# febrianrachmadi/dep-gan-im

Measured on AMD Instinct MI355X. Metric: 2D slices/sec (G+2D+GP train step), 256x256x1 fp32, higher is better.
Workload: dtype f32; 1 GPU; DEP-GAN-IM twoCritics canonical train step (critic-Y2 + critic-DEM + G update, WGAN-GP), batch 32 per GPU, 256x256x1; per_gpu_batch=32, global_batch=32, parallelism=dp1

## Files before the change

dep_gan_im_amd/_lib.py:

```python
from __future__ import annotations

import ctypes as C
import os

HERE = os.path.dirname(os.path.abspath(__file__))
LIB_PATH = os.environ.get("DEPGAN_LIB") or os.path.join(HERE, "libdepgan.so")

EXPORTS = [
    "depgan_last_error", "depgan_create", "depgan_destroy", "depgan_set_stream", "depgan_param_count",
    "depgan_param_info", "depgan_arena_floats", "depgan_arena_ptr", "depgan_weights_changed", "depgan_g_forward",
    "depgan_d_forward", "depgan_critic_grads", "depgan_critic_step", "depgan_g_eval", "depgan_g_grads",
    "depgan_g_step", "depgan_apply_adam", "depgan_last_sums", "depgan_profile_enable", "depgan_profile_read",
    "depgan_profile_reset", "depgan_profile_dump", "depgan_op_conv2d", "depgan_op_conv2d_bwd_data", "depgan_op_conv2d_wgrad",
    "depgan_op_maxpool", "depgan_op_deconv2x2", "depgan_op_deconv2x2_wgrad", "depgan_op_conv2d_stamps", "depgan_uresnet_grads", "depgan_uresnet_step",
    "depgan_uresnet_eval", "depgan_profile_read_bytes", "depgan_g_eval_multi", "depgan_eval_accumulate", "depgan_eval_counts",
    "depgan_data_prep_scratch_floats", "depgan_data_prep_subject", "depgan_abi_version", "depgan_config_size",
    "depgan_set_allreduce", "depgan_get_adam_step", "depgan_set_adam_step", "depgan_gen_iteration", "depgan_eval_divide",
    "depgan_source_hash", "depgan_debug_capture", "depgan_debug_tensor", "depgan_rccl_unique_id", "depgan_rccl_init",
    "depgan_rccl_broadcast", "depgan_rccl_info", "depgan_rccl_shutdown", "depgan_op_conv2d_wgrad_bf16",
    "depgan_op_bn_moments", "depgan_op_bn_backward", "depgan_op_affine_act", "depgan_op_softmax_ce4",
    "depgan_op_bn_rows_fwd", "depgan_op_bn_rows_bwd", "depgan_op_small_gemm",
    "depgan_op_unpool_mask", "depgan_op_gather_pool", "depgan_op_head", "depgan_op_critic_tail_fwd",
    "depgan_op_critic_tail_bwd", "depgan_op_critic_tail_wgrad", "depgan_op_colsum", "depgan_op_sum",
    "depgan_op_critic_inputs", "depgan_op_gp_u0", "depgan_op_critic_stats", "depgan_op_gloss_sums", "depgan_op_g_dpre",
    "depgan_op_film_bwd", "depgan_op_bn_prepare_batch", "depgan_op_bn_gamma_grad_batch", "depgan_op_noise_fwd",
    "depgan_op_noise_bwd", "depgan_op_best_noise", "depgan_op_round_bf16_masked",
    "depgan_data_zscore_scratch_floats", "depgan_data_prep_zscore", "depgan_data_mask_slices", "depgan_labels_to_onehot",
    "depgan_eval_accumulate_channels", "depgan_eval_label_counts",
    "depgan_g_forward_bf16s", "depgan_debug_tensor_bf16s", "depgan_op_conv2d_bf16s", "depgan_op_deconv2x2_bf16s",
    "depgan_op_edge_conv_bf16s", "depgan_op_head_bf16s",
    "depgan_set_fwd_only_storage", "depgan_get_fwd_only_storage", "depgan_op_conv2d_head_bf16s",
    "depgan_set_g_update_storage", "depgan_get_g_update_storage", "depgan_debug_film_decision_bf16s",
    "depgan_op_conv2d_film_train_bf16s", "depgan_op_conv2d_wgrad_bf16s", "depgan_op_conv2d_bwd_data_bf16s",
    "depgan_op_unpool_mask_bf16s", "depgan_op_film_bwd_bf16s", "depgan_op_head_bwd_bf16s",
    "depgan_op_conv2d_fused", "depgan_op_deconv2x2_igemm", "depgan_op_conv2d_wgrad_ex",
    "depgan_set_critic16_pipe", "depgan_get_critic16_pipe", "depgan_op_head_softmax_bf16s",
]

ABI_VERSION = 3
MAX_MULTI, MAX_CRITIC_STEPS = 32, 256
RCCL_ID_BYTES = 128


class Config(C.Structure):
    _fields_ = [("struct_size", C.c_int), ("batch", C.c_int), ("height", C.c_int), ("width", C.c_int),
                ("nicg", C.c_int), ("first_fm", C.c_int), ("im_thresh", C.c_float), ("delta", C.c_float),
                ("lrD", C.c_float), ("lrG", C.c_float), ("beta1", C.c_float), ("beta2", C.c_float),
                ("adam_eps", C.c_float), ("nc_out", C.c_int), ("bf16_weights", C.c_int), ("bf16_mfma", C.c_int),
                ("f32_split", C.c_int)]

    def __init__(self, **kw):
        super().__init__(**kw)
        self.struct_size = C.sizeof(Config)


ALLREDUCE_FN = C.CFUNCTYPE(C.c_int, C.c_void_p, C.c_void_p, C.c_long, C.c_void_p)


NET_G, NET_D_Y2, NET_D_DEM = 0, 1, 2
ARENA_PARAMS, ARENA_NONTRAINABLE, ARENA_GRADS, ARENA_ADAM_M, ARENA_ADAM_V = range(5)

_lib = None


class DepganError(RuntimeError):
    pass


def load():
# ... 99 lines not shown
    lib.depgan_op_g_dpre.argtypes = [vp, i] + [vp] * 5 + [i, L, vp]
    lib.depgan_op_film_bwd.argtypes = [vp] * 4 + [i] + [vp] * 3 + [i, L, i, L, vp]
    lib.depgan_op_bn_prepare_batch.argtypes = [vp, vp, i, f, vp]
    lib.depgan_op_bn_gamma_grad_batch.argtypes = [vp, vp, i, vp]
    lib.depgan_op_noise_fwd.argtypes = [vp] * 6 + [i, vp]
    lib.depgan_op_noise_bwd.argtypes = [vp] * 10 + [i, L, vp]
    lib.depgan_op_best_noise.argtypes = [vp, i, vp, L, vp, vp, vp]
    lib.depgan_op_round_bf16_masked.argtypes = [vp] * 3 + [L, vp]
    lib.depgan_uresnet_grads.argtypes = [vp, vp, vp, vp, C.c_int, C.c_uint, fp]
    lib.depgan_uresnet_step.argtypes = [vp, vp, vp, vp, C.c_int, C.c_uint, fp]
    lib.depgan_uresnet_eval.argtypes = [vp, vp, vp, vp, C.c_int, fp]
    lib.depgan_debug_capture.argtypes = [vp, C.c_int]
    lib.depgan_rccl_unique_id.argtypes = [vp]
    lib.depgan_rccl_init.argtypes = [vp, vp, C.c_int, C.c_int]
    lib.depgan_rccl_broadcast.argtypes = [vp, vp, C.c_long, C.c_int]
    lib.depgan_rccl_info.argtypes = [vp, ip, ip, C.POINTER(C.c_long)]
    lib.depgan_rccl_shutdown.argtypes = [vp]
    lib.depgan_debug_tensor.argtypes = [vp, C.c_char_p, vp, C.c_long, ip]
    lib.depgan_g_forward_bf16s.argtypes = [vp, vp, vp, vp, i]
    lib.depgan_debug_tensor_bf16s.argtypes = [vp, C.c_char_p, vp, L, ip]
    lib.depgan_op_conv2d_bf16s.argtypes = [vp, L, L, L] + [vp] * 6 + [i] + [vp, L, L, L] * 2 + [vp] + [i] * 7 + [vp]
    lib.depgan_op_deconv2x2_bf16s.argtypes = [vp, L, L, L] + [vp] * 4 + [vp, L, L, L] + [i] * 6 + [vp]
    lib.depgan_op_edge_conv_bf16s.argtypes = [vp] * 5 + [vp, L, L, L] + [i] * 6 + [vp]
    lib.depgan_op_head_bf16s.argtypes = [vp] * 4 + [L, i, i, vp]
    lib.depgan_op_head_softmax_bf16s.argtypes = [vp, L] + [vp] * 4 + [L, i, vp]
    lib.depgan_op_conv2d_head_bf16s.argtypes = ([vp, L, L, L] + [vp] * 6 + [i] + [vp, L, L, L] * 2 + [vp] + [i] * 7 +
                                                [vp] * 3 + [i, i, vp])
    lib.depgan_set_fwd_only_storage.argtypes = [vp, i]
    lib.depgan_get_fwd_only_storage.argtypes = [vp]
    lib.depgan_set_g_update_storage.argtypes = [vp, i]
    lib.depgan_get_g_update_storage.argtypes = [vp]
    lib.depgan_set_critic16_pipe.argtypes = [vp, i]
    lib.depgan_get_critic16_pipe.argtypes = [vp]
    lib.depgan_debug_film_decision_bf16s.argtypes = [vp, C.c_char_p, vp, L, ip]
    lib.depgan_op_conv2d_film_train_bf16s.argtypes = ([vp, L, L, L] + [vp] * 6 + [i] + [vp, L, L, L] * 2 + [vp, vp] +
                                                      [i] * 6 + [vp])
    lib.depgan_op_conv2d_wgrad_bf16s.argtypes = [vp, L, L, L] * 2 + [vp, vp] + [i] * 7 + [vp]
    lib.depgan_op_conv2d_bwd_data_bf16s.argtypes = [vp, L, L, L] + [vp] + [vp, L, L, L] * 3 + [i] * 6 + [vp]
    lib.depgan_op_unpool_mask_bf16s.argtypes = [vp, L, L, L] * 4 + [i] * 4 + [vp]
    lib.depgan_op_film_bwd_bf16s.argtypes = [vp] * 4 + [i] + [vp] * 3 + [i, L, i, vp]
    lib.depgan_op_head_bwd_bf16s.argtypes = [i, vp, L] + [vp] * 3 + [L, i, vp]
    lib.depgan_op_conv2d_fused.argtypes = ([vp, L, L, L] + [vp] * 6 + [i] + [vp, L, L, L] * 5 + [vp] * 3 + [i] * 12 +
                                           [vp])
    lib.depgan_op_deconv2x2_igemm.argtypes = [i] + [vp, L, L, L] + [vp] * 4 + [vp, L, L, L] * 2 + [i] * 7 + [vp]
    lib.depgan_op_conv2d_wgrad_ex.argtypes = [vp, L, L, L] * 2 + [vp] * 3 + [i] * 3 + [vp] * 3 + [i] * 7 + [vp]
    _lib = lib
    return lib


def check(rc, what=""):
    if rc != 0:
        msg = load().depgan_last_error()
        raise DepganError("%s failed (status %d): %s" % (what or "libdepgan call", rc,
                                                         msg.decode() if msg else "?"))


_hip = None


def hip():
    global _hip
    if _hip is None:
        last = None
        for name in ("libamdhip64.so", "/opt/rocm/lib/libamdhip64.so", "libamdhip64.so.7", "libamdhip64.so.6"):
            try:
                _hip = C.CDLL(name)
# ... 18 lines not shown
```

dep_gan_im_amd/csrc/common.h:

```cpp
#pragma once
#include <hip/hip_runtime.h>
#include <stdint.h>
#include <stddef.h>

typedef float f32x2 __attribute__((ext_vector_type(2)));
typedef float f32x4 __attribute__((ext_vector_type(4)));
typedef float f32x16 __attribute__((ext_vector_type(16)));

struct TView {
  float* p;
  long sB, sY, sX;
};

static inline TView make_view(float* p, int H, int W, int C) {
  TView v;
  v.p = p;
  v.sX = C;
  v.sY = (long)W * C;
  v.sB = (long)H * W * C;
  return v;
}
static inline TView make_view_slice(float* p, int H, int W, int Ctot, int c0) {
  TView v = make_view(p, H, W, Ctot);
  v.p = p + c0;
// ... 181 lines not shown
  float* dst;
  const float* kscale;
  int ntaps, srcI, srcO, io, transpose, flip;
  int NT, CK, nCC, Kdim, Ndim;
  int bf16;
  int tapg;
  int wino;
  unsigned total;
  unsigned per_nt;
  unsigned nt_stride;
  unsigned blk0, nblk;
};
int dg_pack_job(const ConvPlan& pl, const float* src, int srcI, int srcO, int io, int transpose, int flip,
                const float* kscale, float* dst, size_t nt_stride, PackJob* job);
unsigned dg_pack_layout(PackJob* jobs_host, int njobs);
int dg_pack_weights_batch(const PackJob* jobs_dev, int njobs, unsigned nblocks, hipStream_t st);

int dg_pack_weights(const ConvPlan& pl, const float* src, int srcI, int srcO, int io, int transpose, int flip,
                    const float* kscale, float* dst, hipStream_t st);

int dg_conv_igemm(const ConvPlan& pl, const ConvArgs& a, hipStream_t st);
int dg_conv_igemm_check(const ConvPlan& pl, const ConvArgs& a);
bool dg_conv_igemm_wp_supported(const ConvPlan& pl, const ConvArgs& a, bool force);
int dg_conv_igemm_wp(const ConvPlan& pl, const ConvArgs& a, hipStream_t st);
bool dg_conv_igemm_ws5_supported(const ConvPlan& pl, const ConvArgs& a, bool force);
int dg_conv_igemm_ws5(const ConvPlan& pl, const ConvArgs& a, hipStream_t st);
const char* dg_conv_igemm_ws5_name(const ConvPlan& pl);
int dg_conv_igemm_tile(const ConvPlan& pl, const ConvArgs& a, hipStream_t st);
bool dg_conv_igemm_head_supported(const ConvPlan& pl, const ConvArgs& a);
ConvPlan dg_plan_conv_wino(int Cin, int Cout);
bool dg_conv_wino_supported(const ConvPlan& pl, const ConvArgs& a);
const char* dg_conv_wino_name(const ConvArgs& a);
int dg_conv_wino(const ConvPlan& pl, const ConvArgs& a, hipStream_t st);
void dg_conv_igemm_name(const ConvPlan& pl, const ConvArgs& a, char* buf, size_t cap);
int dg_conv_direct(int KS, const ConvArgs& a, hipStream_t st);

size_t dg_wgrad_part_floats(int KS, int B, int H, int W, int Cin, int Cout);
int dg_wgrad(int KS, const WgradArgs& a, int* nchunks, hipStream_t st);
int dg_wgrad_finish(const float* part, int nchunks, int ntaps, int Cin, int Cout, const float* scale, float* out,
                    float* raw, int accumulate, int oi, const float* colpart, int colC, const float* colscale,
                    float* colout, float* colraw, hipStream_t st);
int dg_wgrad_finish_rows(const float* part, int nchunks, int ntaps, int Cin, int Cout, const float* scale, float* out,
                         float* raw, int accumulate, int oi, const float* colpart, int colrows, int colC,
                         const float* colscale, float* colout, float* colraw, hipStream_t st);
int dg_wgrad_reduce(const float* part, int nchunks, int ntaps, int Cin, int Cout, const float* scale, float* out,
                    float* raw, int accumulate, int oi, hipStream_t st);

bool dg_wgrad_bf16_supported(int KS, int Cin, int Cout);
size_t dg_wgrad_bf16_part_floats(int KS, int B, int H, int W, int Cin, int Cout);
int dg_wgrad_bf16(int KS, const WgradArgs& a, int* nchunks, hipStream_t st);

size_t dg_wgrad_small_part_floats(int KS, int B, int H, int W, int Cin, int Cout);
int dg_wgrad_small(int KS, const WgradArgs& a, int* nchunks, hipStream_t st);
```

dep_gan_im_amd/csrc/igemm_wino.hip:

```cpp
#include <stdlib.h>

#include <type_traits>

#include "common.h"
#include "epilogue.h"

namespace {

constexpr int WN_CK = 8;
constexpr int WN_TW = 18;
constexpr int WN_CP = 36;
constexpr int WN_XV = WN_CK / 4;

template <int MT>
struct WnCfg {
  static constexpr int TH = 8 * MT;
  static constexpr int NTILE = 32 * MT;
  static constexpr int PIXT = (TH + 2) * WN_TW;
  static constexpr int XTOT = PIXT * WN_XV;
  static constexpr int NXP = (XTOT + 255) / 256;
  static constexpr int RAW = NXP * 256 * 4;
  static constexpr int VPLANE = NTILE * WN_CK;
  static constexpr int V = 16 * VPLANE;
  static constexpr int ZPLANE = NTILE * WN_CP + 32;
  static constexpr int Z = 8 * ZPLANE;
  static constexpr size_t LDS = sizeof(float) * (size_t)((2 * RAW + V) > Z ? (2 * RAW + V) : Z);
  static constexpr int WGS_PER_CU = (MT == 2) ? 2 : 3;
};

static __device__ __forceinline__ int rslot(int pix, int half) { return (2 * pix + half) ^ (((pix >> 2) & 1) << 1); }

static __device__ __forceinline__ int vslot(int T, int cg, int a) { return ((2 * T + cg) ^ ((T >> 2) & 1) ^ (a << 1)) << 2; }

template <int MT, bool PERS, bool HEAD, int ABL = 0>
static __device__ __forceinline__ void wino_body(const ConvArgs& a) {
  typedef WnCfg<MT> C;
  constexpr int MF = 32, NT = 32;
  constexpr int WN_RAW = C::RAW, WN_VPLANE = C::VPLANE, WN_ZPLANE = C::ZPLANE, WN_XTOT = C::XTOT, NXP = C::NXP;
  typedef f32x16 acc_t;
  extern __shared__ __attribute__((aligned(16))) float smem[];
  float* const raw0 = smem;
  float* const raw1 = smem + WN_RAW;
  float* V = smem + 2 * WN_RAW;

  const int tid = threadIdx.x;
  const int lane = tid & 63, wv = tid >> 6;
  const int r = lane & 31, h = lane >> 5;
  const int tilesX = (a.W + 15) >> 4, tilesY = (a.H + C::TH - 1) / C::TH;
  const unsigned nNTall = (unsigned)a.lgy, nPix = (unsigned)a.lgx;
  const int nCC = a.Cin / WN_CK;

  constexpr int SENT = (int)0x80000000;
  int xvo[NXP], xyx[NXP];
#pragma unroll
  for (int i = 0; i < NXP; ++i) {
    const int q = tid + i * 256;
    const int lq = q ^ (((q >> 3) & 1) << 1);
    const int pix = lq >> 1, part = lq & 1;
    const int ly = pix / WN_TW, lx = pix - ly * WN_TW;
    xvo[i] = (q < WN_XTOT) ? 4 * (ly * (int)a.in.sY + lx * (int)a.in.sX + part * 4) : SENT;
    xyx[i] = (ly << 8) | lx;
  }
  int tA[MT][4], tB[MT][4], tV[MT];
  float tS[MT];
#pragma unroll
  for (int i = 0; i < MT; ++i) {
    const int q = lane + 64 * i;
    const int cg = q & 1, aa = wv, T = q >> 1;
    const int tyi = T >> 3, txi = T & 7;
    const int rA = (aa == 0) ? 0 : (aa == 2 ? 2 : 1), rB = (aa == 3) ? 3 : (aa == 2 ? 1 : 2);
#pragma unroll
    for (int j = 0; j < 4; ++j) {
      tA[i][j] = 4 * rslot((2 * tyi + rA) * WN_TW + 2 * txi + j, cg);
      tB[i][j] = 4 * rslot((2 * tyi + rB) * WN_TW + 2 * txi + j, cg);
    }
    tV[i] = (4 * aa) * WN_VPLANE + vslot(T, cg, aa);
    tS[i] = (aa == 1) ? 1.f : -1.f;
  }
  const int wbase = __builtin_amdgcn_readfirstlane(wv * 256);
  int aoff[MT];
#pragma unroll
  for (int mt = 0; mt < MT; ++mt) aoff[mt] = vslot(32 * mt + r, h, wv);
  const int boff = (4 * wv * 32 + r) * WN_CK + 4 * h;

  unsigned id = blockIdx.x;
  do {
    int t, ntile;
    if ((nPix & 7u) == 0) {
      const unsigned x = id & 7u, sl = id >> 3;
      ntile = (int)(sl % nNTall);
      t = (int)(x * (nPix >> 3) + sl / nNTall);
    } else {
      t = (int)(id % nPix);
      ntile = (int)(id / nPix);
    }
    const int tx0 = (t % tilesX) * 16;
    t /= tilesX;
    const int ty0 = (t % tilesY) * C::TH;
    const int b = t / tilesY;
    const long out_goff = 0;
    const int n0 = ntile * NT;
    const float* inb = a.in.p + (long)b * a.in.sB;
    const bool interior = ty0 >= 1 && ty0 + C::TH + 1 <= a.H && tx0 >= 1 && tx0 + 17 <= a.W;
    const char* halo0 = reinterpret_cast<const char*>(inb + ((long)(ty0 - 1) * a.in.sY + (long)(tx0 - 1) * a.in.sX));
    auto coff = [&](int cc) -> long {
      if (a.cpt > 0) {
        const int run = cc / a.cpt;
        return a.in_run_off[run] + (long)(cc - run * a.cpt) * WN_CK;
      }
      return (long)cc * WN_CK;
    };
    const float* const xorg = a.in.p - ((long)a.in.sY + (long)a.in.sX);
    const unsigned long long xu = (unsigned long long)xorg;
    const unsigned xlo = __builtin_amdgcn_readfirstlane((unsigned)xu), xhi = __builtin_amdgcn_readfirstlane((unsigned)(xu >> 32));
    const __amdgpu_buffer_rsrc_t rx =
        __builtin_amdgcn_make_buffer_rsrc((void*)(((unsigned long long)xhi << 32) | xlo), 0, 0x7FFFFFFF, 0x00020000);
    const int xso0 = 4 * (b * (int)a.in.sB + ty0 * (int)a.in.sY + tx0 * (int)a.in.sX);
    auto stage_dma = [&](int cc, int buf) {
      const int xso = xso0 + 4 * (int)coff(cc);
      float* xs = (buf ? raw1 : raw0) + wbase;
      if (interior) {
#pragma unroll
        for (int i = 0; i < NXP; ++i) {
          const int vo = xvo[i];
          __builtin_amdgcn_raw_ptr_buffer_load_lds(rx, (__attribute__((address_space(3))) void*)(xs + i * 1024), 16, vo,
                                                   xso, 0, 0);
        }
      } else {
#pragma unroll
        for (int i = 0; i < NXP; ++i) {
          const int iy = ty0 + (xyx[i] >> 8) - 1, ix = tx0 + (xyx[i] & 255) - 1;
          const int vo = (iy >= 0 && iy < a.H && ix >= 0 && ix < a.W) ? xvo[i] : SENT;
          __builtin_amdgcn_raw_ptr_buffer_load_lds(rx, (__attribute__((address_space(3))) void*)(xs + i * 1024), 16, vo,
                                                   xso, 0, 0);
        }
      }
    };

    acc_t acc[4][MT];

    const float* wnt = a.w + (size_t)ntile * nCC * (16 * NT * WN_CK) + boff;
    if (!(ABL & 8)) stage_dma(0, 0);
    auto chunk = [&](const int cc, auto first_tag) {
      constexpr bool FIRST = decltype(first_tag)::value;
      f32x4 bq[4];
#pragma unroll
      for (int f = 0; f < 4; ++f)
        bq[f] = *reinterpret_cast<const f32x4*>(wnt + (size_t)cc * (16 * NT * WN_CK) + f * (NT * WN_CK));
      asm volatile("s_waitcnt vmcnt(0)" ::: "memory");
      __syncthreads();
      if (!(ABL & 8) && cc + 1 < nCC) stage_dma(cc + 1, (cc + 1) & 1);
      const float* raw = (cc & 1) ? raw1 : raw0;
#pragma unroll
      for (int i = 0; i < ((ABL & 2) ? 0 : MT); ++i) {
        f32x4 tc[4];
#pragma unroll
        for (int j = 0; j < 4; ++j) {
          const f32x4 x = *reinterpret_cast<const f32x4*>(raw + tA[i][j]);
          const f32x4 y = *reinterpret_cast<const f32x4*>(raw + tB[i][j]);
#pragma unroll
          for (int k = 0; k < 4; ++k) tc[j][k] = fmaf(y[k], tS[i], x[k]);
        }
        f32x4 v0, v1, v2, v3;
#pragma unroll
        for (int k = 0; k < 4; ++k) {
          v0[k] = tc[0][k] - tc[2][k];
          v1[k] = tc[1][k] + tc[2][k];
          v2[k] = tc[2][k] - tc[1][k];
          v3[k] = tc[1][k] - tc[3][k];
        }
        *reinterpret_cast<f32x4*>(V + tV[i]) = v0;
        *reinterpret_cast<f32x4*>(V + tV[i] + WN_VPLANE) = v1;
        *reinterpret_cast<f32x4*>(V + tV[i] + 2 * WN_VPLANE) = v2;
        *reinterpret_cast<f32x4*>(V + tV[i] + 3 * WN_VPLANE) = v3;
      }
      f32x4 av[2][MT];
      auto load_a = [&](int f, f32x4* d) {
#pragma unroll
        for (int mt = 0; mt < MT; ++mt)
          d[mt] = *reinterpret_cast<const f32x4*>(V + (4 * wv + f) * WN_VPLANE + aoff[mt]);
      };
      load_a(0, av[0]);
#pragma unroll
      for (int f = 0; f < 4; ++f) {
        if (f + 1 < 4) load_a(f + 1, av[(f + 1) & 1]);
        __builtin_amdgcn_sched_barrier(0);
#pragma unroll
        for (int j = 0; j < 4; ++j)
#pragma unroll
          for (int mt = 0; mt < MT; ++mt)
            if (!(ABL & 4)) {
              if (FIRST && j == 0) {
                const acc_t zero = {0.f, 0.f, 0.f, 0.f, 0.f, 0.f, 0.f, 0.f, 0.f, 0.f, 0.f, 0.f, 0.f, 0.f, 0.f, 0.f};
                acc[f][mt] = __builtin_amdgcn_mfma_f32_32x32x2f32(bq[f][j], av[f & 1][mt][j], zero, 0, 0, 0);
              } else {
                acc[f][mt] = __builtin_amdgcn_mfma_f32_32x32x2f32(bq[f][j], av[f & 1][mt][j], acc[f][mt], 0, 0, 0);
              }
            } else {
              if (FIRST && j == 0) acc[f][mt] = acc_t{};
              acc[f][mt][j] += bq[f][j] * av[f & 1][mt][j];
            }
        __builtin_amdgcn_sched_barrier(0);
      }
    };
    chunk(0, std::true_type{});
    for (int cc = 1; cc < nCC; ++cc) chunk(cc, std::false_type{});

    if (ABL & 1) {
      float sacc = 0.f;
#pragma unroll
      for (int f = 0; f < 4; ++f)
#pragma unroll
        for (int mt = 0; mt < MT; ++mt)
#pragma unroll
          for (int j = 0; j < 16; ++j) sacc += acc[f][mt][j];
      if (sacc == 12345.678f) a.out.p[tid] = sacc;
      __syncthreads();
      continue;
    }
    auto zstage = [&]() {
      __syncthreads();
      float* zw = smem + (2 * wv) * WN_ZPLANE + r * WN_CP + 4 * h;
#pragma unroll
      for (int mt = 0; mt < MT; ++mt)
#pragma unroll
        for (int g = 0; g < 4; ++g) {
          f32x4 z0, z1;
#pragma unroll
          for (int k = 0; k < 4; ++k) {
            const float m0 = acc[0][mt][4 * g + k], m1 = acc[1][mt][4 * g + k], m2 = acc[2][mt][4 * g + k],
                        m3 = acc[3][mt][4 * g + k];
            z0[k] = (m0 + m1) + m2;
            z1[k] = (m1 - m2) - m3;
          }
          *reinterpret_cast<f32x4*>(zw + mt * (32 * WN_CP) + 8 * g) = z0;
          *reinterpret_cast<f32x4*>(zw + WN_ZPLANE + mt * (32 * WN_CP) + 8 * g) = z1;
        }
      __syncthreads();
    };
#define EPI_PRE_SYNC
#define EPI_STAGE
#define EPI_STAGE_LATE zstage()
#define EPI_NPASS (4 * MT)
#define EPI_OYW (ty0 + 2 * MT * __builtin_amdgcn_readfirstlane(wv))
#define EPI_FULL ((ty0 + C::TH <= a.H) && (tx0 + 16 <= a.W))
#define EPI_FETCH(v, py, px)                                                                                         \
  {                                                                                                                  \
    const float* zb = smem + ((px)&1) * WN_ZPLANE +                                                                  \
                      ((MT * __builtin_amdgcn_readfirstlane(wv) + ((py) >> 1)) * 8 + ((px) >> 1)) * WN_CP + c4;       \
    const f32x4 za = *reinterpret_cast<const f32x4*>(zb + (((py)&1) ? 2 : 0) * WN_ZPLANE);                           \
    const f32x4 zb1 = *reinterpret_cast<const f32x4*>(zb + (((py)&1) ? 4 : 2) * WN_ZPLANE);                          \
    const f32x4 zc = *reinterpret_cast<const f32x4*>(zb + (((py)&1) ? 6 : 4) * WN_ZPLANE);                           \
    _Pragma("unroll") for (int k_ = 0; k_ < 4; ++k_) v[k_] = ((py)&1) ? (za[k_] - zb1[k_]) - zc[k_] : (za[k_] + zb1[k_]) + zc[k_]; \
  }
#define EPI_HEAD HEAD
#include "igemm_epilogue.inc"
#undef EPI_HEAD
#undef EPI_FETCH
#undef EPI_FULL
#undef EPI_OYW
#undef EPI_NPASS
#undef EPI_STAGE_LATE
#undef EPI_STAGE
#undef EPI_PRE_SYNC
    if (PERS) __syncthreads();
  } while (PERS && (id += gridDim.x) < nPix * nNTall);
}

template <int MT, bool PERS>
__global__ __launch_bounds__(256, WnCfg<MT>::WGS_PER_CU) void wino_conv_kernel(const ConvArgs a) {
  wino_body<MT, PERS, false>(a);
}
template <bool PERS>
__global__ __launch_bounds__(256, 2) void wino_conv_head_kernel(const ConvArgs a) {
  wino_body<2, PERS, true>(a);
}
#ifdef DEPGAN_WINO_ABLATIONS
template <int MT, int ABL>
__global__ __launch_bounds__(256, WnCfg<MT>::WGS_PER_CU) void wino_conv_abl_kernel(const ConvArgs a) {
  wino_body<MT, true, false, ABL>(a);
}
#endif

}

bool dg_conv_wino_supported(const ConvPlan& pl, const ConvArgs& a) {
  if (!dg_plan_wino(pl)) return false;
  if (a.Cin != pl.Cin || (a.Cin % WN_CK) || (a.Cout % 32) || a.groups > 1 || a.dbg || ((a.H | a.W) & 1)) return false;
  if (a.cpt > 0 && ((a.Cin % (a.cpt * WN_CK)) != 0 || a.Cin / (a.cpt * WN_CK) > 4)) return false;
  return true;
}

static int wino_mt(const ConvArgs& a) {
  static int forced = -1;
  if (forced < 0) {
    const char* e = getenv("DEPGAN_WINO_MT");
    forced = e ? atoi(e) : 0;
  }
  if (a.ep.head_out) return 2;
  if (forced == 1 || forced == 2) return forced;
  return 1;
}

template <int MT>
static void wino_geometry(ConvArgs& a, long* total, long* G, bool* pers) {
  a.lgx = cdiv(a.W, 16) * cdiv(a.H, WnCfg<MT>::TH) * a.B;
  a.lgy = a.Cout / 32;
  *total = (long)a.lgx * a.lgy;
  const long cap = (long)WnCfg<MT>::WGS_PER_CU * dg_cu_count();
  *pers = *total > cap;
  *G = *pers ? cap : *total;
}

const char* dg_conv_wino_name(const ConvArgs& a_in) {
  ConvArgs a = a_in;
  long total, G;
  bool pers;
  const int mt = wino_mt(a);
  if (mt == 2) wino_geometry<2>(a, &total, &G, &pers); else wino_geometry<1>(a, &total, &G, &pers);
  if (a.ep.head_out) return pers ? "wino_conv_head_kernel<true>" : "wino_conv_head_kernel<false>";
  if (mt == 2) return pers ? "wino_conv_kernel<2,true>" : "wino_conv_kernel<2,false>";
  return pers ? "wino_conv_kernel<1,true>" : "wino_conv_kernel<1,false>";
}

template <int MT>
static int wino_launch(ConvArgs a, hipStream_t st) {
  long total, G;
  bool pers;
  wino_geometry<MT>(a, &total, &G, &pers);
  constexpr size_t LDS = WnCfg<MT>::LDS;
  static DgOncePerDevice once;
  if (once.need()) {
    HIPCHECK(hipFuncSetAttribute(reinterpret_cast<const void*>(&wino_conv_kernel<MT, false>),
                                 hipFuncAttributeMaxDynamicSharedMemorySize, (int)LDS));
    HIPCHECK(hipFuncSetAttribute(reinterpret_cast<const void*>(&wino_conv_kernel<MT, true>),
                                 hipFuncAttributeMaxDynamicSharedMemorySize, (int)LDS));
    if (MT == 2) {
      HIPCHECK(hipFuncSetAttribute(reinterpret_cast<const void*>(&wino_conv_head_kernel<false>),
                                   hipFuncAttributeMaxDynamicSharedMemorySize, (int)LDS));
      HIPCHECK(hipFuncSetAttribute(reinterpret_cast<const void*>(&wino_conv_head_kernel<true>),
                                   hipFuncAttributeMaxDynamicSharedMemorySize, (int)LDS));
    }
  }
#ifdef DEPGAN_WINO_ABLATIONS
  if (const char* e = getenv("DEPGAN_WINO_ABL")) {
    const int abl = atoi(e);
    if (abl && pers && !a.ep.head_out) {
#define WN_ABL_CASE(N)                                                                                              \
  case N:                                                                                                           \
    HIPCHECK(hipFuncSetAttribute(reinterpret_cast<const void*>(&wino_conv_abl_kernel<MT, N>),                       \
                                 hipFuncAttributeMaxDynamicSharedMemorySize, (int)LDS));                            \
    hipLaunchKernelGGL((wino_conv_abl_kernel<MT, N>), dim3((unsigned)G), dim3(256), LDS, st, a);                    \
    break;
      switch (abl) {
        WN_ABL_CASE(1) WN_ABL_CASE(2) WN_ABL_CASE(3) WN_ABL_CASE(4) WN_ABL_CASE(8) WN_ABL_CASE(10) WN_ABL_CASE(11)
        default: dg_set_error("DEPGAN_WINO_ABL=%d not instantiated", abl); return DG_ERR_ARG;
      }
      HIPCHECK(hipGetLastError());
      return DG_OK;
    }
  }
#endif
  if (a.ep.head_out) {
    if (MT != 2 || a.Cout != 32 || a.ep.pool.p) {
      dg_set_error("dg_conv_wino: the fused head needs 32 output channels and no fused pool");
      return DG_ERR_ARG;
    }
    if (pers) hipLaunchKernelGGL((wino_conv_head_kernel<true>), dim3((unsigned)G), dim3(256), LDS, st, a);
    else hipLaunchKernelGGL((wino_conv_head_kernel<false>), dim3((unsigned)G), dim3(256), LDS, st, a);
  } else {
    if (pers) hipLaunchKernelGGL((wino_conv_kernel<MT, true>), dim3((unsigned)G), dim3(256), LDS, st, a);
    else hipLaunchKernelGGL((wino_conv_kernel<MT, false>), dim3((unsigned)G), dim3(256), LDS, st, a);
  }
  HIPCHECK(hipGetLastError());
  return DG_OK;
}

int dg_conv_wino(const ConvPlan& pl, const ConvArgs& a, hipStream_t st) {
  if (!dg_conv_wino_supported(pl, a)) {
    dg_set_error("dg_conv_wino: shape not covered (3x3, Cin %% 8, Cout %% 32, even H and W, no groups)");
    return DG_ERR_UNSUPPORTED;
  }
  return wino_mt(a) == 2 ? wino_launch<2>(a, st) : wino_launch<1>(a, st);
}
```

dep_gan_im_amd/csrc/op_entries.hip:

```cpp
#include "model.h"
#include "train_ops.h"

#include <math.h>
#include <stdlib.h>
#include <stdio.h>
#include <string.h>

int op_pack_jobs(PackJob* jobs, int n, hipStream_t st) {
  const unsigned nb = dg_pack_layout(jobs, n);
  DevTmp jd(st);
  DGCHECK(jd.alloc(n * sizeof(PackJob)));
  hipError_t e = hipMemcpyAsync(jd.p, jobs, n * sizeof(PackJob), hipMemcpyHostToDevice, st);
  if (e != hipSuccess) { dg_set_error("op_pack_jobs: upload failed: %s", hipGetErrorString(e)); return DG_ERR_HIP; }
  return dg_pack_weights_batch(jd.as<PackJob>(), n, nb, st);
}

extern "C" {

static int op_conv_run(ConvArgs a, const float* w_hwio, int Cin, int Cout, int KS, int path, int bwd, hipStream_t st) {
  const int ci = a.Cin, co = a.Cout;
  ConvPlan pl = (path == 3) ? dg_plan_conv_bf16(KS, ci, co)
                : (path == 4 || path == 5) ? dg_plan_conv_split(KS, ci, co, path == 5 ? 3 : 2)
                : (path == 6) ? dg_plan_conv_items(KS, ci, co, 1L << 30) : dg_plan_conv(KS, ci, co);
  if (path == 7) pl = dg_plan_conv_items(KS, ci, co, 1L << 30);
// ... 27 lines not shown
    if (path == 6 || path == 1) return dg_conv_igemm_tile(pl, a, st);
    return dg_conv_igemm(pl, a, st);
  }
  if (!bwd) conv_set_weights(&a, dg_plan_direct(), nullptr, w_hwio, Cin, Cout);
  else conv_set_weights_bwd(&a, dg_plan_direct(), nullptr, w_hwio, Cin, Cout);
  return dg_conv_direct(KS, a, st);
}

static int op_conv(const float* in, const float* w_hwio, const float* bias, float* out, int B, int H, int W, int Cin,
                   int Cout, int KS, int relu, int path, int bwd, hipStream_t st) {
  const int ci = bwd ? Cout : Cin, co = bwd ? Cin : Cout;
  ConvArgs a = conv_args(make_view(const_cast<float*>(in), H, W, ci), make_view(out, H, W, co), B, H, W, ci, co);
  a.ep.bias = bias;
  a.ep.relu = relu;
  return op_conv_run(a, w_hwio, Cin, Cout, KS, path, bwd, st);
}

int depgan_op_conv2d_stamps(const float* in, const float* w_hwio, float* out, int B, int H, int W, int Cin, int Cout,
                            int KS, unsigned long long* stamps, int reps, void* stream) {
  hipStream_t st = (hipStream_t)stream;
  ConvArgs a = conv_args(make_view(const_cast<float*>(in), H, W, Cin), make_view(out, H, W, Cout), B, H, W, Cin, Cout);
  a.ep.relu = 1;
  ConvPlan pl = dg_plan_conv(KS, Cin, Cout);
  if (!dg_plan_mfma(pl)) { dg_set_error("no MFMA variant"); return DG_ERR_UNSUPPORTED; }
  DevTmp wp(st);
  DGCHECK(wp.alloc(pl.packedFloats * sizeof(float)));
  DGCHECK(dg_pack_weights(pl, w_hwio, Cin, Cout, 0, 0, 0, nullptr, wp.as<float>(), st));
  a.w = wp.as<float>();
  for (int i = 0; i < reps; ++i) {
    a.dbg = (i == reps - 1) ? stamps : nullptr;
    DGCHECK(dg_conv_igemm(pl, a, st));
  }
  return DG_OK;
}

int depgan_op_conv2d(const float* in, const float* w_hwio, const float* bias, float* out, int B, int H, int W,
                     int Cin, int Cout, int KS, int relu, int path, void* stream) {
  return op_conv(in, w_hwio, bias, out, B, H, W, Cin, Cout, KS, relu, path, 0, (hipStream_t)stream);
}
int depgan_op_conv2d_bwd_data(const float* dy, const float* w_hwio, float* dx, int B, int H, int W, int Cin,
                              int Cout, int KS, int path, void* stream) {
  return op_conv(dy, w_hwio, nullptr, dx, B, H, W, Cin, Cout, KS, 0, path, 1, (hipStream_t)stream);
}
int depgan_op_conv2d_wgrad(const float* x, const float* dy, float* dw, int B, int H, int W, int Cin, int Cout, int KS,
                           void* stream) {
  hipStream_t st = (hipStream_t)stream;
  const bool big = (Cin % 4 == 0 && Cout % 4 == 0 && Cin >= 8);
  const size_t pf = big ? dg_wgrad_part_floats(KS, B, H, W, Cin, Cout) : dg_wgrad_small_part_floats(KS, B, H, W, Cin, Cout);
  DevTmp part(st);
  DGCHECK(part.alloc(pf * sizeof(float)));
  WgradArgs a = wgrad_args(make_view(const_cast<float*>(x), H, W, Cin), make_view(const_cast<float*>(dy), H, W, Cout),
                           part.as<float>(), B, H, W, Cin, Cout);
  int nch = 0;
  DGCHECK(big ? dg_wgrad(KS, a, &nch, st) : dg_wgrad_small(KS, a, &nch, st));
  return dg_wgrad_reduce(a.part, nch, KS * KS, Cin, Cout, nullptr, dw, nullptr, 0, 0, st);
}
int depgan_op_conv2d_wgrad_bf16(const float* x, const float* dy, float* dw, int B, int H, int W, int Cin, int Cout,
                                int KS, void* stream) {
  hipStream_t st = (hipStream_t)stream;
  if (!dg_wgrad_bf16_supported(KS, Cin, Cout)) { dg_set_error("op_wgrad_bf16: shape not covered"); return DG_ERR_UNSUPPORTED; }
  const size_t pf = dg_wgrad_bf16_part_floats(KS, B, H, W, Cin, Cout);
  DevTmp part(st);
  DGCHECK(part.alloc(pf * sizeof(float)));
  WgradArgs a = wgrad_args(make_view(const_cast<float*>(x), H, W, Cin), make_view(const_cast<float*>(dy), H, W, Cout),
                           part.as<float>(), B, H, W, Cin, Cout);
  int nch = 0;
// ... 591 lines not shown
```

include/depgan.h:

```cpp
#ifndef DEPGAN_H
#define DEPGAN_H
#include <stddef.h>
#ifdef __cplusplus
extern "C" {
#endif

typedef struct depgan_ctx depgan_ctx;

#define DEPGAN_ABI_VERSION 3
int depgan_abi_version(void);
size_t depgan_config_size(void);
const char* depgan_source_hash(void);

typedef struct depgan_config {
  int struct_size;
  int batch;
  int height;
  int width;
  int nicg;
  int first_fm;
  float im_thresh;
  float delta;
  float lrD, lrG;
  float beta1, beta2, adam_eps;
// ... 143 lines not shown
                                long osY, long osX, void* pool, int B, int H, int W, int Cin, int Cout, int KS, int relu,
                                const float* head_w, const float* head_b, float* head_out, int tanh_act, int skip_out,
                                void* hip_stream);
int depgan_op_deconv2x2_bf16s(const void* in, long isB, long isY, long isX, const float* w_hwoi, const float* bias,
                              const float* scale, const float* shift, void* out, long osB, long osY, long osX, int B,
                              int H, int W, int Cin, int Cout, int relu, void* hip_stream);
int depgan_op_edge_conv_bf16s(const float* in, const float* w_hwio, const float* bias, const float* scale,
                              const float* shift, void* out, long osB, long osY, long osX, int B, int H, int W, int Cin,
                              int Cout, int relu, void* hip_stream);
int depgan_op_head_bf16s(const void* a, const float* w, const float* b, float* out, long P, int C, int tanh_act,
                         void* hip_stream);
int depgan_op_head_softmax_bf16s(const void* a, long ld, const float* w, const float* b, float* probs,
                                 float* logits_or_null, long P, int C, void* hip_stream);

int depgan_op_conv2d(const float* in, const float* w_hwio, const float* bias, float* out, int B, int H, int W,
                     int Cin, int Cout, int KS, int relu, int path, void* hip_stream);
int depgan_op_conv2d_bwd_data(const float* dy, const float* w_hwio, float* dx, int B, int H, int W, int Cin,
                              int Cout, int KS, int path, void* hip_stream);
int depgan_op_conv2d_wgrad(const float* x, const float* dy, float* dw_hwio, int B, int H, int W, int Cin, int Cout,
                           int KS, void* hip_stream);
int depgan_op_conv2d_wgrad_bf16(const float* x, const float* dy, float* dw_hwio, int B, int H, int W, int Cin,
                                int Cout, int KS, void* hip_stream);

int depgan_op_conv2d_stamps(const float* in, const float* w_hwio, float* out, int B, int H, int W, int Cin, int Cout,
                            int KS, unsigned long long* stamps, int reps, void* hip_stream);
int depgan_op_maxpool(const float* in, float* out, int B, int Ho, int Wo, int C, void* hip_stream);
int depgan_op_deconv2x2(const float* in, const float* w_hwoi, const float* bias, const float* scale,
                        const float* shift, float* out, int B, int H, int W, int Cin, int Cout, int relu,
                        void* hip_stream);

int depgan_op_deconv2x2_wgrad(const float* in, const float* dout, float* dw_hwoi, float* colsum, int B, int H, int W,
                              int Cin, int Cout, void* hip_stream);

int depgan_op_conv2d_fused(const float* in, long isB, long isY, long isX, const float* w_hwio, const float* bias,
                           const float* scale, const float* shift, const float* film_mul, const float* film_add,
                           int film_ld, float* out, long osB, long osY, long osX, float* out_pre, long psB, long psY,
                           long psX, const float* res, long rsB, long rsY, long rsX, const float* mask, long msB,
                           long msY, long msX, float* pool, long qsB, long qsY, long qsX, const float* head_w,
                           const float* head_b, float* head_out, int head_tanh, int head_skip_out, int B, int H, int W,
                           int Cin, int Cout, int KS, int relu, int accumulate, int path, int bwd, void* hip_stream);
int depgan_op_deconv2x2_igemm(int form, const float* in, long isB, long isY, long isX, const float* w_hwoi,
                              const float* bias, const float* scale, const float* shift, float* out, long osB, long osY,
                              long osX, const float* mask, long msB, long msY, long msX, int B, int H, int W, int Cin,
                              int Cout, int relu, int path, void* hip_stream);
int depgan_op_conv2d_wgrad_ex(const float* x, long xsB, long xsY, long xsX, const float* dy, long dsB, long dsY,
                              long dsX, const float* scale, float* dw, float* raw, int accumulate, int oi, int colB,
                              const float* colscale, float* colout, float* colraw, int B, int H, int W, int Cin,
                              int Cout, int KS, int bf16, void* hip_stream);

int depgan_op_bn_moments(const float* x, long sB, long sY, long sX, int B, int H, int W, int C, float* mean, float* var,
                         long scratch_floats, void* hip_stream);
int depgan_op_bn_backward(const float* dy, const float* raw, float* draw, long sB, long sY, long sX, int B, int H, int W,
                          int C, const float* gamma, const float* mean, const float* var, float eps, float invN,
                          float dyscale, float* dgamma, float* dbeta, long scratch_floats, void* hip_stream);
int depgan_op_affine_act(const float* in, float* out, float* out_pre, const float* res, long sB, long sY, long sX,
                         const float* s, const float* t, const float* film_mul, const float* film_add, int film_ld,
                         int relu, int B, int H, int W, int C, unsigned drop_seed, float drop_rate, void* hip_stream);
int depgan_op_softmax_ce4(const float* logits, const float* onehot, float* probs, float* dz, float* loss_sum, long P,
                          void* hip_stream);
int depgan_op_bn_rows_fwd(const float* x, float* y, int R, int C, int ld, const float* gamma, const float* beta,
                          float eps, float momentum, float corr, float* moving_mean, float* moving_var, float* mean,
                          float* rstd, int relu, void* hip_stream);
int depgan_op_bn_rows_bwd(const float* dy, const float* x, const float* relu_out, float* dx, int R, int C, int ld,
                          const float* gamma, const float* mean, const float* rstd, float* dgamma, float* dbeta,
                          void* hip_stream);
int depgan_op_small_gemm(int form, const float* A, const float* Bm, const float* bias, float* Cm, int M, int K, int N,
// ... 46 lines not shown
```

Baseline: 652.6 slices/s.

## Compute two output-channel tiles per Winograd workgroup to reuse staged input

Adds a Winograd conv kernel variant where each workgroup computes two 32-channel output tiles, so the transformed input tile staged in LDS is reused across both and loaded half as often. A heuristic picks the variant from channel counts, tile counts and CU occupancy, with an env override and an API knob to force a form. In exchange the kernel holds twice the accumulator registers and has fewer workgroups, which can hurt occupancy and load balance on some shapes.

After: 655.6 slices/s, median of 6. About the same (+0.5%).

```diff
diff --git a/dep_gan_im_amd/_lib.py b/dep_gan_im_amd/_lib.py
--- a/dep_gan_im_amd/_lib.py
+++ b/dep_gan_im_amd/_lib.py
@@ -34,7 +34,7 @@
     "depgan_op_conv2d_film_train_bf16s", "depgan_op_conv2d_wgrad_bf16s", "depgan_op_conv2d_bwd_data_bf16s",
     "depgan_op_unpool_mask_bf16s", "depgan_op_film_bwd_bf16s", "depgan_op_head_bwd_bf16s",
     "depgan_op_conv2d_fused", "depgan_op_deconv2x2_igemm", "depgan_op_conv2d_wgrad_ex",
-    "depgan_set_critic16_pipe", "depgan_get_critic16_pipe", "depgan_op_head_softmax_bf16s",
+    "depgan_set_critic16_pipe", "depgan_get_critic16_pipe", "depgan_op_head_softmax_bf16s", "depgan_wino_form",
 ]
 
 ABI_VERSION = 3
@@ -200,6 +200,7 @@
     lib.depgan_get_g_update_storage.argtypes = [vp]
     lib.depgan_set_critic16_pipe.argtypes = [vp, i]
     lib.depgan_get_critic16_pipe.argtypes = [vp]
+    lib.depgan_wino_form.argtypes = [i]
     lib.depgan_debug_film_decision_bf16s.argtypes = [vp, C.c_char_p, vp, L, ip]
     lib.depgan_op_conv2d_film_train_bf16s.argtypes = ([vp, L, L, L] + [vp] * 6 + [i] + [vp, L, L, L] * 2 + [vp, vp] +
                                                       [i] * 6 + [vp])
diff --git a/dep_gan_im_amd/csrc/common.h b/dep_gan_im_amd/csrc/common.h
--- a/dep_gan_im_amd/csrc/common.h
+++ b/dep_gan_im_amd/csrc/common.h
@@ -237,6 +237,7 @@
 bool dg_conv_wino_supported(const ConvPlan& pl, const ConvArgs& a);
 const char* dg_conv_wino_name(const ConvArgs& a);
 int dg_conv_wino(const ConvPlan& pl, const ConvArgs& a, hipStream_t st);
+int dg_wino_form(int form);
 void dg_conv_igemm_name(const ConvPlan& pl, const ConvArgs& a, char* buf, size_t cap);
 int dg_conv_direct(int KS, const ConvArgs& a, hipStream_t st);
 
diff --git a/dep_gan_im_amd/csrc/igemm_wino.hip b/dep_gan_im_amd/csrc/igemm_wino.hip
--- a/dep_gan_im_amd/csrc/igemm_wino.hip
+++ b/dep_gan_im_amd/csrc/igemm_wino.hip
@@ -32,9 +32,10 @@
 
 static __device__ __forceinline__ int vslot(int T, int cg, int a) { return ((2 * T + cg) ^ ((T >> 2) & 1) ^ (a << 1)) << 2; }
 
-template <int MT, bool PERS, bool HEAD, int ABL = 0>
+template <int MT, bool PERS, bool HEAD, int ABL = 0, int NTW = 1>
 static __device__ __forceinline__ void wino_body(const ConvArgs& a) {
   typedef WnCfg<MT> C;
+  static_assert(NTW == 1 || (NTW == 2 && MT == 1 && !HEAD && ABL == 0), "two channel tiles: 8-row tiles, no fused head");
   constexpr int MF = 32, NT = 32;
   constexpr int WN_RAW = C::RAW, WN_VPLANE = C::VPLANE, WN_ZPLANE = C::ZPLANE, WN_XTOT = C::XTOT, NXP = C::NXP;
   typedef f32x16 acc_t;
@@ -86,20 +87,31 @@
   unsigned id = blockIdx.x;
   do {
     int t, ntile;
+    unsigned idd = id, nNTd = nNTall;
+    int ntoff = 0;
+    if (NTW == 2 && ((a.Cout / NT) & 1)) {
+      nNTd = nNTall - 1;
+      if (id >= nPix * nNTd) {
+        idd = id - nPix * nNTd;
+        ntoff = (int)nNTd;
+        nNTd = 1;
+      }
+    }
     if ((nPix & 7u) == 0) {
-      const unsigned x = id & 7u, sl = id >> 3;
-      ntile = (int)(sl % nNTall);
-      t = (int)(x * (nPix >> 3) + sl / nNTall);
+      const unsigned x = idd & 7u, sl = idd >> 3;
+      ntile = (int)(sl % nNTd) + ntoff;
+      t = (int)(x * (nPix >> 3) + sl / nNTd);
     } else {
-      t = (int)(id % nPix);
-      ntile = (int)(id / nPix);
+      t = (int)(idd % nPix);
+      ntile = (int)(idd / nPix) + ntoff;
     }
     const int tx0 = (t % tilesX) * 16;
     t /= tilesX;
     const int ty0 = (t % tilesY) * C::TH;
     const int b = t / tilesY;
     const long out_goff = 0;
-    const int n0 = ntile * NT;
+    const int nt0 = ntile * NTW;
+    const bool two = NTW == 2 && __builtin_amdgcn_readfirstlane(nt0 + 1) < a.Cout / NT;
     const float* inb = a.in.p + (long)b * a.in.sB;
     const bool interior = ty0 >= 1 && ty0 + C::TH + 1 <= a.H && tx0 >= 1 && tx0 + 17 <= a.W;
     const char* halo0 = reinterpret_cast<const char*>(inb + ((long)(ty0 - 1) * a.in.sY + (long)(tx0 - 1) * a.in.sX));
@@ -137,16 +149,23 @@
       }
     };
 
-    acc_t acc[4][MT];
-
-    const float* wnt = a.w + (size_t)ntile * nCC * (16 * NT * WN_CK) + boff;
+    acc_t acc[NTW][4][MT];
+
+    const float* wnt = a.w + (size_t)nt0 * nCC * (16 * NT * WN_CK) + boff;
+    const size_t wnt1 = (size_t)nCC * (16 * NT * WN_CK);
     if (!(ABL & 8)) stage_dma(0, 0);
-    auto chunk = [&](const int cc, auto first_tag) {
+    auto chunk = [&](const int cc, auto first_tag, auto ntw_tag) {
       constexpr bool FIRST = decltype(first_tag)::value;
-      f32x4 bq[4];
+      constexpr int ntw = decltype(ntw_tag)::value;
+      f32x4 bq[NTW][4];
 #pragma unroll
       for (int f = 0; f < 4; ++f)
-        bq[f] = *reinterpret_cast<const f32x4*>(wnt + (size_t)cc * (16 * NT * WN_CK) + f * (NT * WN_CK));
+        bq[0][f] = *reinterpret_cast<const f32x4*>(wnt + (size_t)cc * (16 * NT * WN_CK) + f * (NT * WN_CK));
+      if (ntw == 2) {
+#pragma unroll
+        for (int f = 0; f < 4; ++f)
+          bq[NTW - 1][f] = *reinterpret_cast<const f32x4*>(wnt + wnt1 + (size_t)cc * (16 * NT * WN_CK) + f * (NT * WN_CK));
+      }
       asm volatile("s_waitcnt vmcnt(0)" ::: "memory");
       __syncthreads();
       if (!(ABL & 8) && cc + 1 < nCC) stage_dma(cc + 1, (cc + 1) & 1);
@@ -189,22 +208,28 @@
         for (int j = 0; j < 4; ++j)
 #pragma unroll
           for (int mt = 0; mt < MT; ++mt)
-            if (!(ABL & 4)) {
-              if (FIRST && j == 0) {
-                const acc_t zero = {0.f, 0.f, 0.f, 0.f, 0.f, 0.f, 0.f, 0.f, 0.f, 0.f, 0.f, 0.f, 0.f, 0.f, 0.f, 0.f};
-                acc[f][mt] = __builtin_amdgcn_mfma_f32_32x32x2f32(bq[f][j], av[f & 1][mt][j], zero, 0, 0, 0);
+#pragma unroll
+            for (int w = 0; w < ntw; ++w)
+              if (!(ABL & 4)) {
+                if (FIRST && j == 0) {
+                  const acc_t zero = {0.f, 0.f, 0.f, 0.f, 0.f, 0.f, 0.f, 0.f, 0.f, 0.f, 0.f, 0.f, 0.f, 0.f, 0.f, 0.f};
+                  acc[w][f][mt] = __builtin_amdgcn_mfma_f32_32x32x2f32(bq[w][f][j], av[f & 1][mt][j], zero, 0, 0, 0);
+                } else {
+                  acc[w][f][mt] = __builtin_amdgcn_mfma_f32_32x32x2f32(bq[w][f][j], av[f & 1][mt][j], acc[w][f][mt], 0, 0, 0);
+                }
               } else {
-                acc[f][mt] = __builtin_amdgcn_mfma_f32_32x32x2f32(bq[f][j], av[f & 1][mt][j], acc[f][mt], 0, 0, 0);
+                if (FIRST && j == 0) acc[w][f][mt] = acc_t{};
+                acc[w][f][mt][j] += bq[w][f][j] * av[f & 1][mt][j];
               }
-            } else {
-              if (FIRST && j == 0) acc[f][mt] = acc_t{};
-              acc[f][mt][j] += bq[f][j] * av[f & 1][mt][j];
-            }
         __builtin_amdgcn_sched_barrier(0);
       }
     };
-    chunk(0, std::true_type{});
-    for (int cc = 1; cc < nCC; ++cc) chunk(cc, std::false_type{});
+    auto chunks = [&](auto ntw_tag) {
+      chunk(0, std::true_type{}, ntw_tag);
+      for (int cc = 1; cc < nCC; ++cc) chunk(cc, std::false_type{}, ntw_tag);
+    };
+    if (NTW == 2 && two) chunks(std::integral_constant<int, NTW>{});
+    else chunks(std::integral_constant<int, 1>{});
 
     if (ABL & 1) {
       float sacc = 0.f;
@@ -213,11 +238,14 @@
 #pragma unroll
         for (int mt = 0; mt < MT; ++mt)
 #pragma unroll
-          for (int j = 0; j < 16; ++j) sacc += acc[f][mt][j];
+          for (int j = 0; j < 16; ++j) sacc += acc[0][f][mt][j];
       if (sacc == 12345.678f) a.out.p[tid] = sacc;
       __syncthreads();
       continue;
     }
+#pragma unroll
+    for (int w = 0; w < NTW; ++w) if (w == 0 || two) {
+    const int n0 = (nt0 + w) * NT;
     auto zstage = [&]() {
       __syncthreads();
       float* zw = smem + (2 * wv) * WN_ZPLANE + r * WN_CP + 4 * h;
@@ -228,8 +256,8 @@
           f32x4 z0, z1;
 #pragma unroll
           for (int k = 0; k < 4; ++k) {
-            const float m0 = acc[0][mt][4 * g + k], m1 = acc[1][mt][4 * g + k], m2 = acc[2][mt][4 * g + k],
-                        m3 = acc[3][mt][4 * g + k];
+            const float m0 = acc[w][0][mt][4 * g + k], m1 = acc[w][1][mt][4 * g + k], m2 = acc[w][2][mt][4 * g + k],
+                        m3 = acc[w][3][mt][4 * g + k];
             z0[k] = (m0 + m1) + m2;
             z1[k] = (m1 - m2) - m3;
           }
@@ -263,6 +291,7 @@
 #undef EPI_STAGE_LATE
 #undef EPI_STAGE
 #undef EPI_PRE_SYNC
+    }
     if (PERS) __syncthreads();
   } while (PERS && (id += gridDim.x) < nPix * nNTall);
 }
@@ -274,6 +303,10 @@
 template <bool PERS>
 __global__ __launch_bounds__(256, 2) void wino_conv_head_kernel(const ConvArgs a) {
   wino_body<2, PERS, true>(a);
+}
+template <bool PERS>
+__global__ __launch_bounds__(256, 2) void wino_conv_nt2_kernel(const ConvArgs a) {
+  wino_body<1, PERS, false, 0, 2>(a);
 }
 #ifdef DEPGAN_WINO_ABLATIONS
 template <int MT, int ABL>
@@ -302,12 +335,33 @@
   return 1;
 }
 
-template <int MT>
+static int g_wino_form = -1;
+
+static int wino_ntw(const ConvArgs& a) {
+  static int env = -2;
+  if (env == -2) {
+    const char* e = getenv("DEPGAN_WINO_NT2");
+    env = e ? atoi(e) : -1;
+  }
+  if (a.ep.head_out || a.Cout < 64 || wino_mt(a) != 1) return 1;
+  if (g_wino_form == 1 || g_wino_form == 2) return g_wino_form;
+  if (env == 0 || env == 1) return env + 1;
+  const int tiles = a.Cout / 32;
+  if (tiles & 1) return 1;
+  if (a.Cin < 64) return 1;
+  const long items = (long)cdiv(a.W, 16) * cdiv(a.H, 8) * a.B * (tiles / 2);
+  const long slots = 2L * dg_cu_count();
+  if (items < slots || (items > slots && items < 2 * slots)) return 1;
+  if (a.Cin == 64 && a.Cout == 64 && items >= 8 * slots) return 1;
+  return 2;
+}
+
+template <int MT, int NTW = 1>
 static void wino_geometry(ConvArgs& a, long* total, long* G, bool* pers) {
   a.lgx = cdiv(a.W, 16) * cdiv(a.H, WnCfg<MT>::TH) * a.B;
-  a.lgy = a.Cout / 32;
+  a.lgy = cdiv(a.Cout / 32, NTW);
   *total = (long)a.lgx * a.lgy;
-  const long cap = (long)WnCfg<MT>::WGS_PER_CU * dg_cu_count();
+  const long cap = (long)(NTW == 2 ? 2 : WnCfg<MT>::WGS_PER_CU) * dg_cu_count();
   *pers = *total > cap;
   *G = *pers ? cap : *total;
 }
@@ -317,6 +371,10 @@
   long total, G;
   bool pers;
   const int mt = wino_mt(a);
+  if (wino_ntw(a) == 2) {
+    wino_geometry<1, 2>(a, &total, &G, &pers);
+    return pers ? "wino_conv_nt2_kernel<true>" : "wino_conv_nt2_kernel<false>";
+  }
   if (mt == 2) wino_geometry<2>(a, &total, &G, &pers); else wino_geometry<1>(a, &total, &G, &pers);
   if (a.ep.head_out) return pers ? "wino_conv_head_kernel<true>" : "wino_conv_head_kernel<false>";
   if (mt == 2) return pers ? "wino_conv_kernel<2,true>" : "wino_conv_kernel<2,false>";
@@ -376,10 +434,35 @@
   return DG_OK;
 }
 
+static int wino_launch_nt2(ConvArgs a, hipStream_t st) {
+  long total, G;
+  bool pers;
+  wino_geometry<1, 2>(a, &total, &G, &pers);
+  constexpr size_t LDS = WnCfg<1>::LDS;
+  static DgOncePerDevice once;
+  if (once.need()) {
+    HIPCHECK(hipFuncSetAttribute(reinterpret_cast<const void*>(&wino_conv_nt2_kernel<false>),
+                                 hipFuncAttributeMaxDynamicSharedMemorySize, (int)LDS));
+    HIPCHECK(hipFuncSetAttribute(reinterpret_cast<const void*>(&wino_conv_nt2_kernel<true>),
+                                 hipFuncAttributeMaxDynamicSharedMemorySize, (int)LDS));
+  }
+  if (pers) hipLaunchKernelGGL((wino_conv_nt2_kernel<true>), dim3((unsigned)G), dim3(256), LDS, st, a);
+  else hipLaunchKernelGGL((wino_conv_nt2_kernel<false>), dim3((unsigned)G), dim3(256), LDS, st, a);
+  HIPCHECK(hipGetLastError());
+  return DG_OK;
+}
+
+int dg_wino_form(int form) {
+  const int prev = g_wino_form;
+  g_wino_form = form;
+  return prev;
+}
+
 int dg_conv_wino(const ConvPlan& pl, const ConvArgs& a, hipStream_t st) {
   if (!dg_conv_wino_supported(pl, a)) {
     dg_set_error("dg_conv_wino: shape not covered (3x3, Cin %% 8, Cout %% 32, even H and W, no groups)");
     return DG_ERR_UNSUPPORTED;
   }
+  if (wino_ntw(a) == 2) return wino_launch_nt2(a, st);
   return wino_mt(a) == 2 ? wino_launch<2>(a, st) : wino_launch<1>(a, st);
 }
diff --git a/dep_gan_im_amd/csrc/op_entries.hip b/dep_gan_im_amd/csrc/op_entries.hip
--- a/dep_gan_im_amd/csrc/op_entries.hip
+++ b/dep_gan_im_amd/csrc/op_entries.hip
@@ -83,6 +83,14 @@
     DGCHECK(dg_conv_igemm(pl, a, st));
   }
   return DG_OK;
+}
+
+int depgan_wino_form(int form) {
+  if (form != -1 && form != 1 && form != 2) {
+    dg_set_error("depgan_wino_form: form must be -1 (the rule), 1 or 2, not %d", form);
+    return -2;
+  }
+  return dg_wino_form(form);
 }
 
 int depgan_op_conv2d(const float* in, const float* w_hwio, const float* bias, float* out, int B, int H, int W,
diff --git a/include/depgan.h b/include/depgan.h
--- a/include/depgan.h
+++ b/include/depgan.h
@@ -199,6 +199,7 @@
 int depgan_op_deconv2x2_wgrad(const float* in, const float* dout, float* dw_hwoi, float* colsum, int B, int H, int W,
                               int Cin, int Cout, void* hip_stream);
 
+int depgan_wino_form(int form);
 int depgan_op_conv2d_fused(const float* in, long isB, long isY, long isX, const float* w_hwio, const float* bias,
                            const float* scale, const float* shift, const float* film_mul, const float* film_add,
                            int film_ld, float* out, long osB, long osY, long osX, float* out_pre, long psB, long psY,
```
